# MobilePerceptionLab/EventCalib

Measured on AMD Instinct MI355X. Metric: Mevents/s DBSCAN+detect, higher is better.
Workload: dtype f64; 1 GPU; ONE 50M-event synthetic circle-grid stream (BASELINE configs[2]'s stream), 346x260, 1 Mev/s, tiled 1.5 ms windows (33334 windows), eps 4 minpts 2; stages: window bounds + EventFrame slicing (reference point order) + DBSCAN(+/-) + circle candidates (reference tie picks); HBM-resident when the timed region starts, upload excluded (reported beside: h2d, ingest); events_total=50000000, events_covered_by_the_ranks_windows=50000000, windows_total=33334, events_per_gpu=50000000, windows_per_gpu=33334, unique_points_per_gpu=38558159, max_window_events=1501, max_segment_points=666, windows_reaching_pairing=26228, circle_candidates=839094, event_point=False

## Files before the change

### eventcalib_amd/csrc/ecal_events.hip

```cpp
#include "ecal_ctx.hpp"
#include "slice_order.hpp"
#include "slice_hash.hpp"

#pragma clang fp contract(off)

namespace ecal {


template <bool STRICT>
__device__ __forceinline__ uint64_t bound_search(const uint8_t *__restrict__ rec, uint64_t n, double t, double t_first, double t_last) {
    auto below = [&](uint64_t i) {
        const double v = load_f64_unaligned(rec + i * RECORD_BYTES);
        return STRICT ? (v <= t) : (v < t);
    };
    if (n == 0) return 0;
    const double f = (t - t_first) / (t_last - t_first);
    uint64_t g = f >= 1.0 ? n - 1 : (f > 0.0 ? (uint64_t) (f * (double) (n - 1)) : 0);
    if (g > n - 1) g = n - 1;
    uint64_t lo, hi;
    if (below(g)) {
        lo = g + 1;
        hi = n;
        for (uint64_t w = 32;; w *= 2) {
            const uint64_t p = g + w;
// ... 422 lines not shown
                                                  uint32_t cap_points, double *__restrict__ xy_out,
                                                  uint32_t *__restrict__ seg_off, uint32_t *__restrict__ seg_cnt,
                                                  int32_t *__restrict__ event_point, int *overflow,
                                                  unsigned char *order_scratch) {
    const uint32_t lo = win_lo[s], n = win_hi[s] - lo, base = win_base[s];
    if (n == 0) {
        if (lo_excl == 0 && threadIdx.x == 0) {
            seg_off[2 * s] = base < cap_points ? base : 0;
            seg_off[2 * s + 1] = seg_off[2 * s];
            seg_cnt[2 * s] = 0;
            seg_cnt[2 * s + 1] = 0;
        }
        return;
    }
    if (n <= lo_excl || n > (uint32_t) CAP) return;
    if ((uint64_t) base + n > cap_points) {
        if (threadIdx.x == 0) {
            *overflow = 1;
            seg_off[2 * s] = seg_off[2 * s + 1] = 0;
            seg_cnt[2 * s] = seg_cnt[2 * s + 1] = 0;
        }
        return;
    }
    using L = SliceLayout<CAP>;
    SliceWork<uint16_t> w;
    w.pts = reinterpret_cast<double2 *>(smem + L::pts_off);
    w.bend = reinterpret_cast<uint32_t *>(smem + L::bend_off);
    w.bend_words = CAP + 4;
    w.pts_words = 4 * CAP;
    w.pos = reinterpret_cast<uint32_t *>(smem + L::pos_off);
    w.sorted = reinterpret_cast<uint16_t *>(smem + L::sorted_off);
    w.rep = reinterpret_cast<uint16_t *>(smem + L::rep_off);
    w.pol = reinterpret_cast<uint8_t *>(smem + L::pol_off);
    w.red = reinterpret_cast<uint32_t *>(smem + L::red_off);
    uint32_t nP, nN;
    OrderScratch ord;
    uint32_t *evk = nullptr;
    if (order_scratch) {
        unsigned char *o = order_scratch + (size_t) blockIdx.x * order_scratch_bytes(CAP);
        order_scratch_carve(o, CAP, &ord, &evk);
    }
    slice_window<T, false, uint16_t>(w, rec, lo, n, Log2c<NB>::value, xy_out + 2 * (size_t) base, event_point ? event_point + base : nullptr,
                                     &nP, &nN, order_scratch ? &ord : nullptr, evk);
    if (threadIdx.x == 0) {
        seg_off[2 * s] = base;
        seg_cnt[2 * s] = nP;
        seg_off[2 * s + 1] = base + nP;
        seg_cnt[2 * s + 1] = nN;
    }
}

template <int CAP, int NB, int T>
__global__ __launch_bounds__(T) void slice_lds_kernel(const uint8_t *__restrict__ rec,
                                                      const uint32_t *__restrict__ win_lo,
                                                      const uint32_t *__restrict__ win_hi,
                                                      const uint32_t *__restrict__ win_base, uint32_t lo_excl,
                                                      uint32_t cap_points, double *__restrict__ xy_out,
                                                      uint32_t *__restrict__ seg_off, uint32_t *__restrict__ seg_cnt,
                                                      int32_t *__restrict__ event_point, int *overflow, uint32_t S,
                                                      const uint32_t *__restrict__ todo,
                                                      const uint32_t *__restrict__ todo_count,
                                                      unsigned char *order_scratch ) {
    extern __shared__ __attribute__((aligned(16))) unsigned char smem[];
    const uint32_t count = todo ? *todo_count : S;
    for (uint32_t k = blockIdx.x; k < count; k += gridDim.x) {
        slice_tier_window<CAP, NB, T>(smem, todo ? todo[k] : k, rec, win_lo, win_hi, win_base, lo_excl, cap_points, xy_out,
                                      seg_off, seg_cnt, event_point, overflow, order_scratch);
        __syncthreads();
    }
}

__global__ void bucket_table_kernel(uint2 *__restrict__ tab) {
    const uint32_t pix = blockIdx.x * blockDim.x + threadIdx.x;
    if (pix >= (1u << 21)) return;
    const uint64_t h = ref_hash_combine2(HASH_INT.v[pix >> 10], HASH_INT.v[pix & 0x3FFu]);
    uint2 w;
    w.x = (uint32_t) (h % 257ull) | ((uint32_t) (h % 541ull) << 9) | ((uint32_t) (h % 1109ull) << 19);
    w.y = (uint32_t) (h % 13ull) | ((uint32_t) (h % 29ull) << 4) | ((uint32_t) (h % 59ull) << 9) | ((uint32_t) (h % 127ull) << 15);
    tab[pix] = w;
}


#ifndef ECAL_RO_WAVES
#define ECAL_RO_WAVES 5
#endif
#if ECAL_RO_WAVES
#define ECAL_RO_ATTR __attribute__((amdgpu_waves_per_eu(ECAL_RO_WAVES, ECAL_RO_WAVES)))
#else
#define ECAL_RO_ATTR
#endif
__global__ __launch_bounds__(PXH_T) ECAL_RO_ATTR void slice_hash_ref_kernel(const uint8_t *__restrict__ rec,
                                                           const uint32_t *__restrict__ win_lo,
                                                           const uint32_t *__restrict__ win_hi,
                                                           const uint32_t *__restrict__ win_base, uint32_t cap_points,
                                                           double *__restrict__ xy_out, uint32_t *__restrict__ seg_off,
                                                           uint32_t *__restrict__ seg_cnt,
                                                           int32_t *__restrict__ event_point, int *overflow,
                                                           uint32_t *__restrict__ todo,
                                                           uint32_t *__restrict__ todo_count,
                                                           const uint2 *__restrict__ bucket_tab, uint32_t *__restrict__ xy16,
                                                           uint32_t *__restrict__ seg_fmt) {
    extern __shared__ __attribute__((aligned(16))) unsigned char smem[];
    slice_hash_window<11, true>(smem, blockIdx.x, rec, win_lo, win_hi, win_base, cap_points, xy_out, seg_off, seg_cnt, event_point, overflow,
                                todo, todo_count, bucket_tab, xy16, seg_fmt);
}

__global__ __launch_bounds__(PXH_T) void slice_hash_kernel(const uint8_t *__restrict__ rec,
                                                           const uint32_t *__restrict__ win_lo,
                                                           const uint32_t *__restrict__ win_hi,
                                                           const uint32_t *__restrict__ win_base, uint32_t cap_points,
                                                           double *__restrict__ xy_out, uint32_t *__restrict__ seg_off,
                                                           uint32_t *__restrict__ seg_cnt,
                                                           int32_t *__restrict__ event_point, int *overflow,
                                                           uint32_t *__restrict__ todo,
                                                           uint32_t *__restrict__ todo_count, uint32_t *__restrict__ xy16,
                                                           uint32_t *__restrict__ seg_fmt) {
    extern __shared__ __attribute__((aligned(16))) unsigned char smem[];
    slice_hash_window<11, false>(smem, blockIdx.x, rec, win_lo, win_hi, win_base, cap_points, xy_out, seg_off, seg_cnt, event_point, overflow,
                                 todo, todo_count, nullptr, xy16, seg_fmt);
}

template <bool THIRD >
__global__ __launch_bounds__(PXH_T) __attribute__((amdgpu_waves_per_eu(THIRD ? 2 : 3, THIRD ? 2 : 3))) void slice_hash_ref_both_kernel(const uint8_t *__restrict__ rec, const uint32_t *__restrict__ win_lo,
                                                                    const uint32_t *__restrict__ win_hi, const uint32_t *__restrict__ win_base,
                                                                    uint32_t cap_points, double *__restrict__ xy_out, uint32_t *__restrict__ seg_off,
                                                                    uint32_t *__restrict__ seg_cnt, int32_t *__restrict__ event_point, int *overflow,
                                                                    uint32_t *__restrict__ todo, uint32_t *__restrict__ todo_count,
                                                                    uint32_t *__restrict__ todo2, uint32_t *__restrict__ todo2_count,
                                                                    uint32_t *__restrict__ todo3, uint32_t *__restrict__ todo3_count,
                                                                    const uint2 *__restrict__ bucket_tab, uint32_t *__restrict__ xy16,
                                                                    uint32_t *__restrict__ seg_fmt) {
    extern __shared__ __attribute__((aligned(16))) unsigned char smem[];
    const uint32_t s = blockIdx.x;
    const uint32_t n = win_hi[s] - win_lo[s];
    if constexpr (THIRD) {
        bool done = false;
        if (n <= PixHash<11>::CAP)
            done = slice_hash_window<11, true>(smem, s, rec, win_lo, win_hi, win_base, cap_points, xy_out, seg_off, seg_cnt, event_point, overflow,
                                               nullptr, nullptr, bucket_tab, xy16, seg_fmt);
        if (!done && n <= PixHash<12>::CAP) {
            __syncthreads();
            done = slice_hash_window<12, true>(smem, s, rec, win_lo, win_hi, win_base, cap_points, xy_out, seg_off, seg_cnt, event_point, overflow,
                                               nullptr, nullptr, bucket_tab, xy16, seg_fmt);
        }
        if (!done) {
            __syncthreads();
            slice_hash_window<13, true>(smem, s, rec, win_lo, win_hi, win_base, cap_points, xy_out, seg_off, seg_cnt, event_point, overflow, todo3,
                                        todo3_count, bucket_tab, xy16, seg_fmt);
        }
        return;
    }
    if (n <= PixHash<11>::CAP)
        slice_hash_window<11, true>(smem, s, rec, win_lo, win_hi, win_base, cap_points, xy_out, seg_off, seg_cnt, event_point, overflow, todo,
                                    todo_count, bucket_tab, xy16, seg_fmt);
    else
        slice_hash_window<12, true>(smem, s, rec, win_lo, win_hi, win_base, cap_points, xy_out, seg_off, seg_cnt, event_point, overflow, todo2,
                                    todo2_count, bucket_tab, xy16, seg_fmt);
}

__global__ __launch_bounds__(PXH_T) __attribute__((amdgpu_waves_per_eu(2, 2))) void slice_hash_third_kernel(const uint8_t *__restrict__ rec, const uint32_t *__restrict__ win_lo,
                                                                 const uint32_t *__restrict__ win_hi, const uint32_t *__restrict__ win_base,
                                                                 uint32_t cap_points, double *__restrict__ xy_out, uint32_t *__restrict__ seg_off,
                                                                 uint32_t *__restrict__ seg_cnt, int32_t *__restrict__ event_point, int *overflow,
                                                                 uint32_t *__restrict__ todo, uint32_t *__restrict__ todo_count,
                                                                 const uint32_t *__restrict__ in_list, const uint32_t *__restrict__ in_count,
                                                                 const uint2 *__restrict__ bucket_tab, uint32_t *__restrict__ xy16,
                                                                 uint32_t *__restrict__ seg_fmt) {
// ... 407 lines not shown
```

### eventcalib_amd/csrc/slice_hash.hpp

```cpp
#pragma once
#include "ecal_ctx.hpp"
#include "slice_order.hpp"

#pragma clang fp contract(off)

namespace ecal {

constexpr int RECORD_BYTES = 25;

__device__ __forceinline__ double load_f64_unaligned(const uint8_t *p) {
    double v;
    __builtin_memcpy(&v, p, 8);
    return v;
}

#ifdef ECAL_PHASE_PROF
static __device__ unsigned long long g_ro_cycles[16];
#define RO_MARK(i)                                                                                  \
    do {                                                                                            \
        if (REFORDER && LOGC == 11 && threadIdx.x == 0) {                                           \
            const unsigned long long now__ = __builtin_amdgcn_s_memtime();                          \
            atomicAdd(&g_ro_cycles[i], now__ - ro_t__);                                             \
            ro_t__ = now__;                                                                         \
        }                                                                                           \
    } while (0)
#else
#define RO_MARK(i)
#endif
#ifndef ECAL_RO_STOP
#define ECAL_RO_STOP 0
#endif
#ifndef ECAL_SL_STOP
#define ECAL_SL_STOP 0
#endif

constexpr int PXH_T = 256;
#ifndef ECAL_PXH13_PER
#define ECAL_PXH13_PER 20
#endif
template <int LOGC>
struct PixHash {
    static constexpr uint32_t SLOTS = 1u << LOGC;
    static constexpr int PER = LOGC == 13 ? ECAL_PXH13_PER : (int) (SLOTS / PXH_T);
    static constexpr uint32_t CAP = (uint32_t) PER * PXH_T - 1u;
    static constexpr uint32_t PIXB = 32u - LOGC;
    static constexpr double XMAX = (double) ((1u << (PIXB - 10u)) - 1u), YMAX = 1023.0;
    static constexpr size_t tab_off = 0;
    static constexpr size_t red_off = tab_off + 8 * SLOTS;
    static constexpr size_t bytes = red_off + 16 * 8 + 16;
    static __device__ __forceinline__ uint32_t slot(uint32_t pix) { return (pix * 0x9E3779B1u) >> (32u - LOGC); }
#ifndef ECAL_RO_NI
#define ECAL_RO_NI 9
#endif
#ifndef ECAL_RO_NI2
#define ECAL_RO_NI2 16
#endif
    static constexpr int NI = LOGC == 11 ? ECAL_RO_NI : (LOGC == 12 ? ECAL_RO_NI2 : 19);
    static constexpr int MAX_EPOCHS = LOGC == 11 ? 7 : 8;
    static constexpr uint32_t NOFF = 128u * NI, PSL = 2u * NOFF;
#ifndef ECAL_RO_FA
#define ECAL_RO_FA 2400
#endif
    static constexpr uint32_t FA_CAP = LOGC == 11 ? (uint32_t) ECAL_RO_FA : 4800u;
    static constexpr size_t w_off = 0;
    static constexpr size_t region_off = w_off + 4 * PSL;
    static constexpr size_t cur_off = region_off + 2 * (PSL > SLOTS ? PSL : SLOTS);
    static constexpr size_t fa_off = cur_off + 2 * PSL;
    static constexpr size_t keep_off = fa_off + 4 * FA_CAP;
    static constexpr size_t bcnt_off = keep_off + 4 * 16 * NI;
    static constexpr size_t ored_off = bcnt_off + 4 * (SLOTS / 64 + 4);
    static constexpr size_t obytes = ored_off + 16 * 8 + 16;
};

struct HashIntTable {
    uint64_t v[2048];
    constexpr HashIntTable() : v{} {
        for (int i = 0; i < 2048; i++) v[i] = ref_hash_f64_bits(__builtin_bit_cast(uint64_t, (double) i));
    }
};
static __device__ const HashIntTable HASH_INT = HashIntTable();

struct ModB {
    double b, inv;
};
__host__ __device__ constexpr double ref_step_inv(int e) { return (1.0 / (double) ref_bucket_step(e)) * (1.0 - 0x1p-50); }
struct StepInvTable {
    double inv[12];
    constexpr StepInvTable() : inv{} {
        for (int e = 0; e < 12; e++) inv[e] = ref_step_inv(e);
    }
};
__device__ __forceinline__ ModB mod_for_epoch(int e) {
    constexpr StepInvTable tabl = StepInvTable();
    ModB m;
    m.b = (double) ref_bucket_step(e);
    m.inv = tabl.inv[e];
    return m;
}
__device__ __forceinline__ double mod_step(double v, const ModB m) {
    const double q = __builtin_trunc(v * m.inv);
    double r = __builtin_fma(-q, m.b, v);
    if (r >= m.b) r -= m.b;
    return r;
}
__device__ __forceinline__ uint32_t mod_hash(uint64_t h, const ModB m) {
    const double d1 = (double) (uint32_t) (h >> 40);
    const double d0 = __builtin_fma((double) (uint32_t) ((h >> 32) & 0xFFu), 0x1p32, (double) (uint32_t) h);
    const double r1 = mod_step(d1, m);
    return (uint32_t) mod_step(__builtin_fma(r1, 0x1p40, d0), m);
}

__device__ __forceinline__ void lds_barrier() {
    asm volatile("s_waitcnt lgkmcnt(0)\n\ts_barrier" ::: "memory");
}

__device__ __forceinline__ void wave_sync_lds() {
    __builtin_amdgcn_fence(__ATOMIC_ACQ_REL, "wavefront");
    __builtin_amdgcn_wave_barrier();
}

__device__ __forceinline__ uint32_t wave_incl_scan_dpp(uint32_t x) {
    uint32_t t = x;
    t += (uint32_t) __builtin_amdgcn_update_dpp(0, (int) x, 0x111, 0xF, 0xF, false);
    t += (uint32_t) __builtin_amdgcn_update_dpp(0, (int) x, 0x112, 0xF, 0xF, false);
    t += (uint32_t) __builtin_amdgcn_update_dpp(0, (int) x, 0x113, 0xF, 0xF, false);
    t += (uint32_t) __builtin_amdgcn_update_dpp(0, (int) t, 0x114, 0xF, 0xE, false);
    t += (uint32_t) __builtin_amdgcn_update_dpp(0, (int) t, 0x118, 0xF, 0xC, false);
    t += (uint32_t) __builtin_amdgcn_update_dpp(0, (int) t, 0x142, 0xA, 0xF, false);
    t += (uint32_t) __builtin_amdgcn_update_dpp(0, (int) t, 0x143, 0xC, 0xF, false);
    return t;
}

__device__ __forceinline__ void early_epochs_packed(uint32_t m, uint32_t *fa, uint32_t *W, uint16_t *region, uint16_t *cur_out) {
    const uint32_t lane = threadIdx.x & 63u;
    const uint32_t m_e = m < 127u ? m : 127u;
    uint32_t bw[2], cur[2] = {0u, 0u};
#pragma unroll
    for (int i = 0; i < 2; i++) bw[i] = (lane + 64u * i < m_e) ? fa[lane + 64u * i] : 0u;
    wave_sync_lds();
    uint32_t n_prev = 0;
    for (int e = 0; e < 4 && n_prev < m_e; e++) {
        const uint32_t B = (uint32_t) ref_bucket_step(e);
        const uint32_t n_e = m_e < B ? m_e : B;
        const uint32_t sh = e == 0 ? 0u : (e == 1 ? 4u : (e == 2 ? 9u : 15u)), mask = (16u << e) - 1u;
#pragma unroll
        for (int i = 0; i < 2; i++) {
            if (lane + 64u * i < B) fa[lane + 64u * i] = 0xFFFFFFFFu;
            if (lane + 64u * i < m_e) W[lane + 64u * i] = 0u;
        }
        wave_sync_lds();
        uint32_t b[2], q[2], f[2], sl[2];
#pragma unroll
        for (int i = 0; i < 2; i++) {
            const uint32_t u = lane + 64u * i;
            q[i] = u < n_prev ? cur[i] : u;
            b[i] = (bw[i] >> sh) & mask;
            if (u < n_e) atomicMin(&fa[b[i]], q[i]);
        }
        wave_sync_lds();
#pragma unroll
        for (int i = 0; i < 2; i++) {
            const uint32_t u = lane + 64u * i;
            f[i] = 0;
            sl[i] = 0;
            if (u < n_e) {
                f[i] = fa[b[i]];
                sl[i] = atomicAdd(&W[f[i]], 1u);
            }
        }
        wave_sync_lds();
        {
            const uint32_t c0 = 2u * lane < n_e ? W[2u * lane] : 0u, c1 = 2u * lane + 1u < n_e ? W[2u * lane + 1u] : 0u;
            const uint32_t ex = wave_incl_scan_dpp(c0 + c1) - c0 - c1;
            if (2u * lane < n_e) W[2u * lane] = (ex << 16) | c0;
            if (2u * lane + 1u < n_e) W[2u * lane + 1u] = ((ex + c0) << 16) | c1;
        }
        wave_sync_lds();
#pragma unroll
        for (int i = 0; i < 2; i++) {
            const uint32_t u = lane + 64u * i;
            if (u < n_e) region[(W[f[i]] >> 16) + sl[i]] = (uint16_t) q[i];
        }
        wave_sync_lds();
#pragma unroll
        for (int i = 0; i < 2; i++) {
            const uint32_t u = lane + 64u * i;
            if (u < n_e) {
                const uint32_t w = W[f[i]], b0 = w >> 16, c = w & 0xFFFFu;
                uint32_t within = 0;
                for (uint32_t t = 0; t < c; t++) within += ((uint32_t) region[b0 + t] < q[i]) ? 1u : 0u;
                cur[i] = n_e - 1u - (b0 + within);
            }
        }
        wave_sync_lds();
        n_prev = n_e;
    }
#pragma unroll
    for (int i = 0; i < 2; i++)
        if (lane + 64u * i < m_e) cur_out[lane + 64u * i] = (uint16_t) cur[i];
}

template <int LOGC, bool REFORDER>
__device__ __forceinline__ bool slice_hash_window(unsigned char *smem, const uint32_t s, const uint8_t *__restrict__ rec,
                                                  const uint32_t *__restrict__ win_lo, const uint32_t *__restrict__ win_hi,
                                                  const uint32_t *__restrict__ win_base, uint32_t cap_points,
                                                  double *__restrict__ xy_out, uint32_t *__restrict__ seg_off,
                                                  uint32_t *__restrict__ seg_cnt, int32_t *__restrict__ event_point,
                                                  int *overflow, uint32_t *__restrict__ todo,
                                                  uint32_t *__restrict__ todo_count, const uint2 *__restrict__ bucket_tab = nullptr,
                                                  uint32_t *__restrict__ xy16 = nullptr, uint32_t *__restrict__ seg_fmt = nullptr) {
    using L = PixHash<LOGC>;
    constexpr int T = PXH_T;
#ifdef ECAL_PHASE_PROF
    unsigned long long ro_t__ = __builtin_amdgcn_s_memtime();
#endif
    constexpr uint32_t PXH_CAP = L::CAP, PXH_SLOTS = L::SLOTS, IDXM = L::SLOTS - 1u, PIXB = L::PIXB;
    constexpr uint32_t MB = LOGC <= 12 ? 12u : 13u, M_IDX = (1u << MB) - 1u, M_ER = 1u << MB, M_POL = 2u << MB, M_KEY = 4u << MB;
    static_assert(MB + 3u <= 16u && L::CAP <= M_IDX, "the word's fields");
    constexpr int PXH_PER = L::PER;
    constexpr uint32_t NONE = L::CAP, EMPTY = 0xFFFFFFFFu;
    const uint32_t tid = threadIdx.x;
    const uint32_t lo = win_lo[s], n = win_hi[s] - lo, base = win_base[s];
    if (n == 0) {
        if (tid == 0) {
            seg_off[2 * s] = base < cap_points ? base : 0;
            seg_off[2 * s + 1] = seg_off[2 * s];
            seg_cnt[2 * s] = 0;
            seg_cnt[2 * s + 1] = 0;
            if (seg_fmt) seg_fmt[2 * s] = seg_fmt[2 * s + 1] = 0u;
        }
        return true;
    }
    if (n > PXH_CAP) {
        if (tid == 0) {
            if (todo) todo[atomicAdd(todo_count, 1u)] = s;
            if (seg_fmt) seg_fmt[2 * s] = seg_fmt[2 * s + 1] = 0u;
        }
        return false;
    }
    if ((uint64_t) base + n > cap_points) {
        if (tid == 0) {
            *overflow = 1;
            seg_off[2 * s] = seg_off[2 * s + 1] = 0;
            seg_cnt[2 * s] = seg_cnt[2 * s + 1] = 0;
            if (seg_fmt) seg_fmt[2 * s] = seg_fmt[2 * s + 1] = 0u;
        }
        return true;
    }
    uint32_t *const tab = reinterpret_cast<uint32_t *>(smem + L::tab_off);
    uint16_t *const pos = reinterpret_cast<uint16_t *>(smem + L::tab_off);
    uint32_t *const red = reinterpret_cast<uint32_t *>(smem + L::red_off);
    uint32_t *const badf = red + 32;

    double vx[PXH_PER], vy[PXH_PER];
    uint32_t vp[PXH_PER];
#pragma unroll
    for (int j = 0; j < PXH_PER; j++) {
        const uint32_t k = tid + j * T;
        vx[j] = 0;
        vy[j] = 0;
        vp[j] = 0;
        if (k < n) {
            const uint8_t *r = rec + (uint64_t) (lo + k) * RECORD_BYTES;
            vx[j] = load_f64_unaligned(r + 8);
            vy[j] = load_f64_unaligned(r + 16);
            vp[j] = r[24];
        }
    }
    {
        uint4 *t4 = reinterpret_cast<uint4 *>(tab);
        for (uint32_t q = tid; q < 2 * PXH_SLOTS / 4; q += T) t4[q] = make_uint4(EMPTY, EMPTY, EMPTY, EMPTY);
    }
    bool bad = false;
    uint32_t pix[PXH_PER];
#pragma unroll
    for (int j = 0; j < PXH_PER; j++) {
        const uint32_t k = tid + j * T;
        const double x = vx[j], y = vy[j];
        const bool okc = x == floor(x) && y == floor(y) && x <= L::XMAX && y <= L::YMAX && __double_as_longlong(x) >= 0 &&
                         __double_as_longlong(y) >= 0;
        bad = bad || (k < n && !okc);
        pix[j] = (((uint32_t) (int) x << 10) | ((uint32_t) (int) y & 0x3FFu)) & ((1u << PIXB) - 1u);
    }
    const bool wave_bad = __any(bad);
    if ((tid & 63) == 0) badf[tid >> 6] = wave_bad ? 1u : 0u;
    __syncthreads();
    if (badf[0] | badf[1] | badf[2] | badf[3]) {
        if (tid == 0) {
            if (todo) todo[atomicAdd(todo_count, 1u)] = s;
            if (seg_fmt) seg_fmt[2 * s] = seg_fmt[2 * s + 1] = 0u;
        }
        return false;
    }
    if (ECAL_SL_STOP == 1) return true;
    constexpr bool EARLY_GATHER = REFORDER;
    uint2 bw[EARLY_GATHER ? PXH_PER : 1];
    if constexpr (EARLY_GATHER) {
#pragma unroll
        for (int j = 0; j < PXH_PER; j++) bw[j] = (tid + j * T < n) ? bucket_tab[pix[j]] : make_uint2(0u, 0u);
    }
    uint32_t hs[PXH_PER];
    {
        uint32_t w0[PXH_PER];
#pragma unroll
        for (int j = 0; j < PXH_PER; j++) {
            hs[j] = L::slot(pix[j]);
            w0[j] = tab[(vp[j] ? PXH_SLOTS : 0u) + hs[j]];
        }
#pragma unroll
        for (int j = 0; j < PXH_PER; j++) {
            const uint32_t k = tid + j * T;
            if (k < n) {
                uint32_t *const t = tab + (vp[j] ? PXH_SLOTS : 0u);
                const uint32_t mine = (pix[j] << LOGC) | k;
                uint32_t h = hs[j], w = w0[j];
                for (;;) {
                    if (w == EMPTY) w = atomicCAS(&t[h], EMPTY, mine);
                    if (w == EMPTY) break;
                    if ((w >> LOGC) == pix[j]) {
                        atomicMin(&t[h], mine);
                        break;
                    }
                    h = (h + 1u) & (PXH_SLOTS - 1u);
                    w = t[h];
                }
                hs[j] = h;
            }
        }
    }
    if constexpr (EARLY_GATHER) lds_barrier(); else __syncthreads();
    if (ECAL_SL_STOP == 2) return true;
    uint32_t repk[PXH_PER];
    uint32_t firstk[PXH_PER];
    {
        uint32_t fw[PXH_PER], ow[PXH_PER];
#pragma unroll
        for (int j = 0; j < PXH_PER; j++) {
            fw[j] = tab[(vp[j] ? PXH_SLOTS : 0u) + hs[j]];
            ow[j] = tab[(vp[j] ? 0u : PXH_SLOTS) + L::slot(pix[j])];
        }
#pragma unroll
        for (int j = 0; j < PXH_PER; j++) {
            const uint32_t k = tid + j * T;
            if (k < n) {
                const uint32_t first = fw[j] & IDXM;
                const uint32_t *const o = tab + (vp[j] ? 0u : PXH_SLOTS);
                uint32_t h = L::slot(pix[j]), w = ow[j];
                bool both = false;
                for (;;) {
                    if (w == EMPTY) break;
                    if ((w >> LOGC) == pix[j]) {
                        both = true;
                        break;
                    }
                    h = (h + 1u) & (PXH_SLOTS - 1u);
                    w = o[h];
                }
                repk[j] = both ? NONE : first;
                firstk[j] = first | (both ? 0x8000u : 0u);
            } else {
                repk[j] = NONE;
                firstk[j] = 0xFFFFu;
            }
        }
    }
    if constexpr (EARLY_GATHER) lds_barrier(); else __syncthreads();
    RO_MARK(1);
    if (ECAL_SL_STOP == 3) return true;
    if constexpr (REFORDER) {
        constexpr uint32_t N_EARLY = 127u;
        uint32_t *const W = reinterpret_cast<uint32_t *>(smem + L::w_off);
        uint16_t *const region = reinterpret_cast<uint16_t *>(smem + L::region_off);
        uint16_t *const cur = reinterpret_cast<uint16_t *>(smem + L::cur_off);
        uint32_t *const fa = reinterpret_cast<uint32_t *>(smem + L::fa_off);
        uint32_t *const keepW = reinterpret_cast<uint32_t *>(smem + L::keep_off);
        uint32_t *const ored = reinterpret_cast<uint32_t *>(smem + L::ored_off);
        uint16_t *const posE = region;
        const uint32_t lane = tid & 63u, wave = tid >> 6;
        constexpr uint32_t NBATCH = (uint32_t) PXH_PER * (T / 64);
        uint32_t *const bcnt = reinterpret_cast<uint32_t *>(smem + L::bcnt_off);
        uint32_t meta[PXH_PER];
#pragma unroll
        for (int j = 0; j < PXH_PER; j++) {
            const uint32_t k = tid + j * T;
            const bool isu = k < n && (firstk[j] & 0x7FFFu) == k;
            const unsigned long long mP = __ballot(isu && vp[j] != 0), mN = __ballot(isu && vp[j] == 0);
            const unsigned long long lower = (1ull << lane) - 1ull;
            const uint32_t below = (uint32_t) __popcll((vp[j] ? mP : mN) & lower);
            if (lane == 0) bcnt[j * (T / 64) + wave] = (uint32_t) __popcll(mP) | ((uint32_t) __popcll(mN) << 16);
            meta[j] = k < n ? ((firstk[j] & M_IDX) | ((firstk[j] & 0x8000u) ? M_ER : 0u) | (vp[j] ? M_POL : 0u) |
                               (isu ? M_KEY : 0u) | (below << 16))
                            : M_ER;
        }
        if constexpr (EARLY_GATHER) lds_barrier(); else __syncthreads();
    RO_MARK(2);
        if (tid < 64u) {
            if constexpr (NBATCH <= 64u) {
                const uint32_t v = tid < NBATCH ? bcnt[tid] : 0u;
                uint32_t inc = v;
#pragma unroll
                for (int d = 1; d < 64; d <<= 1) {
                    const uint32_t o = __shfl_up(inc, d, 64);
                    if (lane >= (uint32_t) d) inc += o;
                }
                if (tid < NBATCH) bcnt[tid] = inc - v;
                if (tid == 63u) bcnt[NBATCH] = inc;
            } else {
                static_assert(NBATCH <= 128u, "two batches per lane");
                const uint32_t v0 = 2u * tid < NBATCH ? bcnt[2u * tid] : 0u, v1 = 2u * tid + 1u < NBATCH ? bcnt[2u * tid + 1u] : 0u;
                uint32_t inc = v0 + v1;
#pragma unroll
                for (int d = 1; d < 64; d <<= 1) {
                    const uint32_t o = __shfl_up(inc, d, 64);
                    if (lane >= (uint32_t) d) inc += o;
                }
                if (2u * tid < NBATCH) bcnt[2u * tid] = inc - v0 - v1;
                if (2u * tid + 1u < NBATCH) bcnt[2u * tid + 1u] = inc - v1;
                if (tid == 63u) bcnt[NBATCH] = inc;
            }
        }
        if constexpr (EARLY_GATHER) lds_barrier(); else __syncthreads();
    RO_MARK(3);
        const uint32_t totals = bcnt[NBATCH], mP = totals & 0xFFFFu, mN = totals >> 16;
        const int EP = mP ? ref_epochs(mP) : 0, EN = mN ? ref_epochs(mN) : 0;
        {
            const uint32_t need = (EP ? (uint32_t) ref_bucket_step(EP - 1) : 0u) + (EN ? (uint32_t) ref_bucket_step(EN - 1) : 0u);
            if (need > L::FA_CAP || EP > L::MAX_EPOCHS || EN > L::MAX_EPOCHS || mP > 128u * (uint32_t) L::NI ||
                mN > 128u * (uint32_t) L::NI) {
                if (tid == 0) {
            if (todo) todo[atomicAdd(todo_count, 1u)] = s;
            if (seg_fmt) seg_fmt[2 * s] = seg_fmt[2 * s + 1] = 0u;
        }
                return false;
            }
        }
        {
            constexpr int NI = L::NI;
            const uint32_t faN = EP ? (uint32_t) ref_bucket_step(EP - 1) : 0u;
            {
#pragma unroll
                for (int j = 0; j < PXH_PER; j++) {
                    const uint32_t ex = bcnt[j * (T / 64) + wave];
                    meta[j] += ((meta[j] & M_POL) ? (ex & 0xFFFFu) : (ex >> 16)) << 16;
                    if (meta[j] & M_KEY) {
                        const uint32_t rank = meta[j] >> 16;
                        const bool pos_ = (meta[j] & M_POL) != 0;
                        W[(pos_ ? 0u : L::NOFF) + rank] = bw[j].x | ((meta[j] & M_ER) ? 0x80000000u : 0u);
                        if (rank < N_EARLY) fa[(pos_ ? 0u : faN) + rank] = bw[j].y;
                        if (L::MAX_EPOCHS > 7 && (pos_ ? EP : EN) > 7)
                            region[(pos_ ? 0u : L::NOFF) + rank] =
                                (uint16_t) mod_hash(ref_hash_combine2(HASH_INT.v[pix[j] >> 10], HASH_INT.v[pix[j] & 0x3FFu]), mod_for_epoch(7));
                    }
                }
            }
            if (ECAL_RO_STOP == 2) return true;
            const uint32_t pol = __builtin_amdgcn_readfirstlane(wave >> 1), sub = __builtin_amdgcn_readfirstlane(wave & 1u);
            const uint32_t l128 = lane + 64u * sub;
            const uint32_t m = pol == 0u ? mP : mN;
            const int E = pol == 0u ? EP : EN;
            const uint32_t uoff = pol == 0u ? 0u : L::NOFF;
            uint32_t *const Wp = W + uoff, *const fap = fa + (pol == 0u ? 0u : faN);
            uint16_t *const regp = region + uoff, *const curp = cur + uoff;
            constexpr uint32_t KW = 4u * NI;
            uint32_t *const kW = keepW + pol * KW, *const kPre = keepW + 2u * KW + pol * KW;
            if (tid == 0) ored[10] = 0u;
            __syncthreads();
    RO_MARK(4);
            uint32_t bk[NI], cu[NI];
#pragma unroll
            for (int i = 0; i < NI; i++) {
                const uint32_t u = l128 + 128u * i;
                bk[i] = u < m ? Wp[u] : 0u;
                cu[i] = (L::MAX_EPOCHS > 7 && E > 7 && u < m) ? ((uint32_t) regp[u] << 16) : 0u;
            }
            if (l128 < KW) kW[l128] = 0u;
            __syncthreads();
    RO_MARK(5);
            if (sub == 0u && m) early_epochs_packed(m, fap, Wp, regp, curp);
            __syncthreads();
    RO_MARK(6);
            if (ECAL_RO_STOP == 3) return true;
            if (l128 < (m < 127u ? m : 127u)) cu[0] = (cu[0] & 0xFFFF0000u) | (uint32_t) curp[l128];
            const int EMAX = EP > EN ? EP : EN;
            if (E > 4) {
                for (uint32_t b = l128; b < 257u; b += 128u) fap[b] = 0xFFFFFFFFu;
            }
            __syncthreads();
    RO_MARK(7);
            for (int e = 4; e < EMAX; e++) {
                const bool on = e < E;
                const uint32_t B = (uint32_t) ref_bucket_step(e), Bprev = (uint32_t) ref_bucket_step(e - 1);
                const uint32_t n_e = on ? (m < B ? m : B) : 0u;
                const uint32_t sh = e == 4 ? 0u : (e == 5 ? 9u : (e == 6 ? 19u : 16u)),
                               bmask = e == 4 ? 0x1FFu : (e == 5 ? 0x3FFu : (e == 6 ? 0x7FFu : 0xFFFu));
                const bool e7 = e == 7;
                const uint32_t per = (n_e + 127u) >> 7;
                uint32_t fq[NI];
                for (uint32_t t = 0; t < per; t++) Wp[l128 + 128u * t] = 0u;
#pragma unroll
                for (int i = 0; i < NI; i++) {
                    const uint32_t u = l128 + 128u * i;
                    if (128u * i >= n_e) break;
                    if (u < n_e) atomicMin(&fap[((e7 ? cu[i] : bk[i]) >> sh) & bmask], u < Bprev ? (cu[i] & 0xFFFFu) : u);
                }
                __syncthreads();
#pragma unroll
                for (int i = 0; i < NI; i++) {
                    const uint32_t u = l128 + 128u * i;
                    fq[i] = 0u;
                    if (128u * i >= n_e) break;
                    if (u < n_e) {
                        const uint32_t f = fap[((e7 ? cu[i] : bk[i]) >> sh) & bmask];
                        fq[i] = f | (atomicAdd(&Wp[f], 1u) << 12);
                    }
                }
                __syncthreads();
                {
                    uint32_t c[NI], sum = 0, big = 0;
#pragma unroll
                    for (int t = 0; t < NI; t++) {
                        c[t] = 0u;
                        if ((uint32_t) t < per) c[t] = Wp[l128 * per + t];
                        sum += c[t];
                        big |= c[t];
                    }
                    if (__any(big > 1023u)) ored[10] = 1u;
                    const uint32_t inc = wave_incl_scan_dpp(sum);
                    if (lane == 63u) ored[wave] = inc;
                    uint32_t ex = inc - sum;
#pragma unroll
                    for (int t = 0; t < NI; t++) {
                        if ((uint32_t) t < per) Wp[l128 * per + t] = (ex << 10) | (c[t] & 0x3FFu);
                        ex += c[t];
                    }
                    if (e + 1 < E) {
                        const uint32_t Bn = (uint32_t) ref_bucket_step(e + 1);
                        for (uint32_t b = l128; b < Bn; b += 128u) fap[b] = 0xFFFFFFFFu;
                    }
                }
                __syncthreads();
                const uint32_t carry_from = 64u * per, carry = __builtin_amdgcn_readfirstlane(ored[pol * 2u]);
#pragma unroll
                for (int i = 0; i < NI; i++) {
                    const uint32_t u = l128 + 128u * i;
                    if (128u * i >= n_e) break;
                    if (u < n_e) {
                        const uint32_t f = fq[i] & 0xFFFu, w = Wp[f];
                        if ((w & 0x3FFu) > 2u)
                            regp[(w >> 10) + (f >= carry_from ? carry : 0u) + (fq[i] >> 12)] = (uint16_t) (u < Bprev ? (cu[i] & 0xFFFFu) : u);
                    }
                }
                __syncthreads();
#pragma unroll
                for (int i = 0; i < NI; i++) {
                    const uint32_t u = l128 + 128u * i;
                    if (128u * i >= n_e) break;
                    if (u < n_e) {
                        const uint32_t f = fq[i] & 0xFFFu, w = Wp[f], b0 = (w >> 10) + (f >= carry_from ? carry : 0u), cnt = w & 0x3FFu;
                        const uint32_t q = u < Bprev ? (cu[i] & 0xFFFFu) : u;
                        uint32_t within = (q != f) ? 1u : 0u;
                        if (cnt > 2u) {
                            const uint32_t r0 = regp[b0], r1 = regp[b0 + 1u], r2 = regp[b0 + 2u], r3 = regp[b0 + 3u];
                            within = (r0 < q ? 1u : 0u) + (r1 < q ? 1u : 0u) + (r2 < q ? 1u : 0u) + ((cnt > 3u && r3 < q) ? 1u : 0u);
                            for (uint32_t t = 4; t < cnt; t++) within += ((uint32_t) regp[b0 + t] < q) ? 1u : 0u;
                        }
                        cu[i] = (cu[i] & 0xFFFF0000u) | (n_e - 1u - (b0 + within));
                    }
                }
                __syncthreads();
                RO_MARK(8 + (e - 4));
            }
            if (ECAL_RO_STOP == 4) return true;
            if (ored[10]) {
                if (tid == 0) {
            if (todo) todo[atomicAdd(todo_count, 1u)] = s;
            if (seg_fmt) seg_fmt[2 * s] = seg_fmt[2 * s + 1] = 0u;
        }
                return false;
            }
#pragma unroll
            for (int i = 0; i < NI; i++) {
                const uint32_t u = l128 + 128u * i;
                if (u < m && !(bk[i] >> 31)) atomicOr(&kW[(cu[i] & 0xFFFFu) >> 5], 1u << (cu[i] & 31u));
            }
            __syncthreads();
    RO_MARK(11);
            if (sub == 0u) {
                static_assert(KW <= 128u, "two bitmap words per lane");
                const uint32_t c0 = 2u * lane < KW ? (uint32_t) __popc(kW[2u * lane]) : 0u;
                const uint32_t c1 = 2u * lane + 1u < KW ? (uint32_t) __popc(kW[2u * lane + 1u]) : 0u;
                const uint32_t inc = wave_incl_scan_dpp(c0 + c1);
                if (2u * lane < KW) kPre[2u * lane] = inc - c0 - c1;
                if (2u * lane + 1u < KW) kPre[2u * lane + 1u] = inc - c1;
                if (lane == 63u) ored[8u + pol] = inc;
            }
            __syncthreads();
    RO_MARK(12);
#pragma unroll
            for (int i = 0; i < NI; i++) {
                const uint32_t u = l128 + 128u * i;
                if (u < m && !(bk[i] >> 31))
                    curp[u] = (uint16_t) (kPre[(cu[i] & 0xFFFFu) >> 5] + (uint32_t) __popc(kW[(cu[i] & 0xFFFFu) >> 5] & ((1u << (cu[i] & 31u)) - 1u)));
            }
            __syncthreads();
    RO_MARK(13);
            const uint32_t nP = mP ? __builtin_amdgcn_readfirstlane(ored[8]) : 0u, nN = mN ? __builtin_amdgcn_readfirstlane(ored[9]) : 0u;
            const bool want_ep = event_point != nullptr;
            if (want_ep) {
#pragma unroll
                for (int j = 0; j < PXH_PER; j++) {
                    if ((meta[j] & (M_KEY | M_ER)) == M_KEY)
                        posE[meta[j] & M_IDX] = cur[((meta[j] & M_POL) ? 0u : L::NOFF) + (meta[j] >> 16)];
                }
                __syncthreads();
            }
    RO_MARK(14);
            double2 *out2 = reinterpret_cast<double2 *>(xy_out) + base;
            int32_t *ep = want_ep ? event_point + base : nullptr;
#pragma unroll
            for (int j = 0; j < PXH_PER; j++) {
                const uint32_t k = tid + j * T;
                if (k < n) {
                    if (meta[j] & M_ER) {
                        if (want_ep) ep[k] = -1;
                    } else if (want_ep || (meta[j] & M_KEY)) {
                        const uint32_t at = want_ep ? posE[meta[j] & M_IDX]
                                                    : (uint32_t) cur[((meta[j] & M_POL) ? 0u : L::NOFF) + (meta[j] >> 16)];
                        if (want_ep) ep[k] = (int32_t) at;
                        if (meta[j] & M_KEY) {
                            const uint32_t slot = (meta[j] & M_POL) ? at : nP + at;
                            if (xy16) {
                                xy16[base + slot] = (pix[j] >> 10) | ((pix[j] & 0x3FFu) << 16);
                            } else {
                                double2 v;
                                v.x = (double) (pix[j] >> 10);
                                v.y = (double) (pix[j] & 0x3FFu);
                                out2[slot] = v;
                            }
                        }
                    }
                }
            }
            if (tid == 0) {
                seg_off[2 * s] = base;
                seg_cnt[2 * s] = nP;
                seg_off[2 * s + 1] = base + nP;
                seg_cnt[2 * s + 1] = nN;
                if (seg_fmt) seg_fmt[2 * s] = seg_fmt[2 * s + 1] = xy16 ? 1u : 0u;
            }
            RO_MARK(15);
            RO_MARK(0);
            return true;
        }
    }
    constexpr uint32_t NBATCH = (uint32_t) PXH_PER * (T / 64);
    static_assert(REFORDER || NBATCH <= 64u, "the canonical-order form scans one batch per lane (first and second pass only)");
    uint32_t *const bcnt = tab + PXH_SLOTS;
    const uint32_t lane = tid & 63u, wave = tid >> 6;
    uint32_t below[PXH_PER];
#pragma unroll
    for (int j = 0; j < PXH_PER; j++) {
        const uint32_t k = tid + j * T;
        const bool isrep = k < n && repk[j] == k;
        const unsigned long long mP = __ballot(isrep && vp[j] != 0), mN = __ballot(isrep && vp[j] == 0);
        const unsigned long long lower = (1ull << lane) - 1ull;
        below[j] = (uint32_t) __popcll((vp[j] ? mP : mN) & lower);
        if (lane == 0) bcnt[j * (T / 64) + wave] = (uint32_t) __popcll(mP) | ((uint32_t) __popcll(mN) << 16);
    }
    __syncthreads();
    if (tid < 64u) {
        const uint32_t v = tid < NBATCH ? bcnt[tid] : 0u;
        uint32_t inc = v;
#pragma unroll
        for (int d = 1; d < 64; d <<= 1) {
            const uint32_t o = __shfl_up(inc, d, 64);
            if (lane >= (uint32_t) d) inc += o;
        }
        if (tid < NBATCH) bcnt[tid] = inc - v;
        if (tid == 63u) bcnt[NBATCH] = inc;
    }
    __syncthreads();
    const uint32_t totals = bcnt[NBATCH], nP = totals & 0xFFFFu, nN = totals >> 16;
#pragma unroll
    for (int j = 0; j < PXH_PER; j++) {
        const uint32_t k = tid + j * T;
        if (k < n && repk[j] == k) {
            const uint32_t ex = bcnt[j * (T / 64) + wave];
            pos[k] = (uint16_t) ((vp[j] ? (ex & 0xFFFFu) : (ex >> 16)) + below[j]);
        }
    }
    __syncthreads();
    if (ECAL_SL_STOP == 4) return true;
    double2 *out2 = reinterpret_cast<double2 *>(xy_out) + base;
    int32_t *ep = event_point ? event_point + base : nullptr;
#pragma unroll
    for (int j = 0; j < PXH_PER; j++) {
        const uint32_t k = tid + j * T;
        if (k < n) {
            const uint32_t r = repk[j];
            if (r == NONE) {
                if (ep) ep[k] = -1;
            } else {
                const uint32_t at = pos[r];
                if (ep) ep[k] = (int32_t) at;
                if (r == k) {
                    const uint32_t slot = vp[j] ? at : nP + at;
                    if (xy16) {
                        xy16[base + slot] = (pix[j] >> 10) | ((pix[j] & 0x3FFu) << 16);
                    } else {
                        double2 v;
                        v.x = (double) (pix[j] >> 10);
                        v.y = (double) (pix[j] & 0x3FFu);
                        out2[slot] = v;
                    }
                }
            }
        }
    }
    if (tid == 0) {
        seg_off[2 * s] = base;
        seg_cnt[2 * s] = nP;
        seg_off[2 * s + 1] = base + nP;
        seg_cnt[2 * s + 1] = nN;
        if (seg_fmt) seg_fmt[2 * s] = seg_fmt[2 * s + 1] = xy16 ? 1u : 0u;
    }
    return true;
}
}
```

Measured before the change: 20010 Mevents/s.

## Raise slice pass occupancy: alias LDS buffers, pack polarity, add short-window form

Pushes the first slicing pass from five to six waves per EU and shrinks its LDS footprint so six workgroups fit per CU. The cur array now aliases the W buffer, and the early-epoch positions are placed inside W. Polarity is packed into bit 31 of the pixel word, and two meta slots are stashed to LDS across the long epoch section, both to cut register pressure. A short-form specialization with fewer per-thread slots handles windows under 6*T events. The aliasing is only safe if cur and W lifetimes never overlap, and the stash adds LDS traffic.

```diff
diff --git a/eventcalib_amd/csrc/ecal_events.hip b/eventcalib_amd/csrc/ecal_events.hip
--- a/eventcalib_amd/csrc/ecal_events.hip
+++ b/eventcalib_amd/csrc/ecal_events.hip
@@ -528,7 +528,7 @@
 
 
 #ifndef ECAL_RO_WAVES
-#define ECAL_RO_WAVES 5
+#define ECAL_RO_WAVES 6
 #endif
 #if ECAL_RO_WAVES
 #define ECAL_RO_ATTR __attribute__((amdgpu_waves_per_eu(ECAL_RO_WAVES, ECAL_RO_WAVES)))
diff --git a/eventcalib_amd/csrc/slice_hash.hpp b/eventcalib_amd/csrc/slice_hash.hpp
--- a/eventcalib_amd/csrc/slice_hash.hpp
+++ b/eventcalib_amd/csrc/slice_hash.hpp
@@ -64,13 +64,19 @@
     static constexpr uint32_t FA_CAP = LOGC == 11 ? (uint32_t) ECAL_RO_FA : 4800u;
     static constexpr size_t w_off = 0;
     static constexpr size_t region_off = w_off + 4 * PSL;
-    static constexpr size_t cur_off = region_off + 2 * (PSL > SLOTS ? PSL : SLOTS);
-    static constexpr size_t fa_off = cur_off + 2 * PSL;
+    static constexpr size_t cur_off = w_off;
+    static constexpr size_t ecur_off = 4 * 128;
+    static_assert(ecur_off + 2 * 128 <= 4 * NOFF, "the early epochs' positions lie inside the set's part of W");
+    static_assert(cur_off + 2 * PSL <= region_off, "cur lies inside W (every LOGC): nothing sits between region and fa any more");
+    static constexpr size_t fa_off = region_off + 2 * (PSL > SLOTS ? PSL : SLOTS);
     static constexpr size_t keep_off = fa_off + 4 * FA_CAP;
     static constexpr size_t bcnt_off = keep_off + 4 * 16 * NI;
     static constexpr size_t ored_off = bcnt_off + 4 * (SLOTS / 64 + 4);
-    static constexpr size_t obytes = ored_off + 16 * 8 + 16;
+    static constexpr int NSTASH = LOGC == 11 ? 2 : 0, STASH0 = 4;
+    static constexpr size_t stash_off = ored_off + 16 * 8 + 16;
+    static constexpr size_t obytes = stash_off + 4 * NSTASH * PXH_T;
 };
+static_assert(6 * PixHash<11>::obytes <= 163840 && PixHash<11>::obytes <= 27136, "first pass: six workgroups per CU");
 
 struct HashIntTable {
     uint64_t v[2048];
@@ -200,15 +206,15 @@
         if (lane + 64u * i < m_e) cur_out[lane + 64u * i] = (uint16_t) cur[i];
 }
 
-template <int LOGC, bool REFORDER>
-__device__ __forceinline__ bool slice_hash_window(unsigned char *smem, const uint32_t s, const uint8_t *__restrict__ rec,
-                                                  const uint32_t *__restrict__ win_lo, const uint32_t *__restrict__ win_hi,
-                                                  const uint32_t *__restrict__ win_base, uint32_t cap_points,
-                                                  double *__restrict__ xy_out, uint32_t *__restrict__ seg_off,
-                                                  uint32_t *__restrict__ seg_cnt, int32_t *__restrict__ event_point,
-                                                  int *overflow, uint32_t *__restrict__ todo,
-                                                  uint32_t *__restrict__ todo_count, const uint2 *__restrict__ bucket_tab = nullptr,
-                                                  uint32_t *__restrict__ xy16 = nullptr, uint32_t *__restrict__ seg_fmt = nullptr) {
+template <int LOGC, bool REFORDER, int PER>
+__device__ __forceinline__ bool slice_hash_window_slots(unsigned char *smem, const uint32_t s, const uint8_t *__restrict__ rec,
+                                                        const uint32_t *__restrict__ win_lo, const uint32_t *__restrict__ win_hi,
+                                                        const uint32_t *__restrict__ win_base, uint32_t cap_points,
+                                                        double *__restrict__ xy_out, uint32_t *__restrict__ seg_off,
+                                                        uint32_t *__restrict__ seg_cnt, int32_t *__restrict__ event_point,
+                                                        int *overflow, uint32_t *__restrict__ todo,
+                                                        uint32_t *__restrict__ todo_count, const uint2 *__restrict__ bucket_tab,
+                                                        uint32_t *__restrict__ xy16, uint32_t *__restrict__ seg_fmt) {
     using L = PixHash<LOGC>;
     constexpr int T = PXH_T;
 #ifdef ECAL_PHASE_PROF
@@ -217,7 +223,8 @@
     constexpr uint32_t PXH_CAP = L::CAP, PXH_SLOTS = L::SLOTS, IDXM = L::SLOTS - 1u, PIXB = L::PIXB;
     constexpr uint32_t MB = LOGC <= 12 ? 12u : 13u, M_IDX = (1u << MB) - 1u, M_ER = 1u << MB, M_POL = 2u << MB, M_KEY = 4u << MB;
     static_assert(MB + 3u <= 16u && L::CAP <= M_IDX, "the word's fields");
-    constexpr int PXH_PER = L::PER;
+    static_assert(PER >= 1 && PER <= L::PER, "a short form of the pass: fewer slots, the same tables and limits");
+    constexpr int PXH_PER = PER;
     constexpr uint32_t NONE = L::CAP, EMPTY = 0xFFFFFFFFu;
     const uint32_t tid = threadIdx.x;
     const uint32_t lo = win_lo[s], n = win_hi[s] - lo, base = win_base[s];
@@ -271,6 +278,10 @@
         uint4 *t4 = reinterpret_cast<uint4 *>(tab);
         for (uint32_t q = tid; q < 2 * PXH_SLOTS / 4; q += T) t4[q] = make_uint4(EMPTY, EMPTY, EMPTY, EMPTY);
     }
+    constexpr uint32_t POLB = 0x80000000u, PIXM = (1u << PIXB) - 1u;
+    static_assert(PIXB < 31u, "bit 31 of the pixel word is free");
+#define PIX_OF(w) ((w) & PIXM)
+#define POL_OF(w) (((w) & POLB) != 0u)
     bool bad = false;
     uint32_t pix[PXH_PER];
 #pragma unroll
@@ -280,7 +291,7 @@
         const bool okc = x == floor(x) && y == floor(y) && x <= L::XMAX && y <= L::YMAX && __double_as_longlong(x) >= 0 &&
                          __double_as_longlong(y) >= 0;
         bad = bad || (k < n && !okc);
-        pix[j] = (((uint32_t) (int) x << 10) | ((uint32_t) (int) y & 0x3FFu)) & ((1u << PIXB) - 1u);
+        pix[j] = ((((uint32_t) (int) x << 10) | ((uint32_t) (int) y & 0x3FFu)) & PIXM) | (vp[j] ? POLB : 0u);
     }
     const bool wave_bad = __any(bad);
     if ((tid & 63) == 0) badf[tid >> 6] = wave_bad ? 1u : 0u;
@@ -297,27 +308,27 @@
     uint2 bw[EARLY_GATHER ? PXH_PER : 1];
     if constexpr (EARLY_GATHER) {
 #pragma unroll
-        for (int j = 0; j < PXH_PER; j++) bw[j] = (tid + j * T < n) ? bucket_tab[pix[j]] : make_uint2(0u, 0u);
+        for (int j = 0; j < PXH_PER; j++) bw[j] = (tid + j * T < n) ? bucket_tab[PIX_OF(pix[j])] : make_uint2(0u, 0u);
     }
     uint32_t hs[PXH_PER];
     {
         uint32_t w0[PXH_PER];
 #pragma unroll
         for (int j = 0; j < PXH_PER; j++) {
-            hs[j] = L::slot(pix[j]);
-            w0[j] = tab[(vp[j] ? PXH_SLOTS : 0u) + hs[j]];
+            hs[j] = L::slot(PIX_OF(pix[j]));
+            w0[j] = tab[(POL_OF(pix[j]) ? PXH_SLOTS : 0u) + hs[j]];
         }
 #pragma unroll
         for (int j = 0; j < PXH_PER; j++) {
             const uint32_t k = tid + j * T;
             if (k < n) {
-                uint32_t *const t = tab + (vp[j] ? PXH_SLOTS : 0u);
+                uint32_t *const t = tab + (POL_OF(pix[j]) ? PXH_SLOTS : 0u);
                 const uint32_t mine = (pix[j] << LOGC) | k;
                 uint32_t h = hs[j], w = w0[j];
                 for (;;) {
                     if (w == EMPTY) w = atomicCAS(&t[h], EMPTY, mine);
                     if (w == EMPTY) break;
-                    if ((w >> LOGC) == pix[j]) {
+                    if ((w >> LOGC) == PIX_OF(pix[j])) {
                         atomicMin(&t[h], mine);
                         break;
                     }
@@ -336,20 +347,20 @@
         uint32_t fw[PXH_PER], ow[PXH_PER];
 #pragma unroll
         for (int j = 0; j < PXH_PER; j++) {
-            fw[j] = tab[(vp[j] ? PXH_SLOTS : 0u) + hs[j]];
-            ow[j] = tab[(vp[j] ? 0u : PXH_SLOTS) + L::slot(pix[j])];
+            fw[j] = tab[(POL_OF(pix[j]) ? PXH_SLOTS : 0u) + hs[j]];
+            ow[j] = tab[(POL_OF(pix[j]) ? 0u : PXH_SLOTS) + L::slot(PIX_OF(pix[j]))];
         }
 #pragma unroll
         for (int j = 0; j < PXH_PER; j++) {
             const uint32_t k = tid + j * T;
             if (k < n) {
                 const uint32_t first = fw[j] & IDXM;
-                const uint32_t *const o = tab + (vp[j] ? 0u : PXH_SLOTS);
-                uint32_t h = L::slot(pix[j]), w = ow[j];
+                const uint32_t *const o = tab + (POL_OF(pix[j]) ? 0u : PXH_SLOTS);
+                uint32_t h = L::slot(PIX_OF(pix[j])), w = ow[j];
                 bool both = false;
                 for (;;) {
                     if (w == EMPTY) break;
-                    if ((w >> LOGC) == pix[j]) {
+                    if ((w >> LOGC) == PIX_OF(pix[j])) {
                         both = true;
                         break;
                     }
@@ -384,11 +395,12 @@
         for (int j = 0; j < PXH_PER; j++) {
             const uint32_t k = tid + j * T;
             const bool isu = k < n && (firstk[j] & 0x7FFFu) == k;
-            const unsigned long long mP = __ballot(isu && vp[j] != 0), mN = __ballot(isu && vp[j] == 0);
+            const bool pol_ = POL_OF(pix[j]);
+            const unsigned long long mP = __ballot(isu && pol_), mN = __ballot(isu && !pol_);
             const unsigned long long lower = (1ull << lane) - 1ull;
-            const uint32_t below = (uint32_t) __popcll((vp[j] ? mP : mN) & lower);
+            const uint32_t below = (uint32_t) __popcll((pol_ ? mP : mN) & lower);
             if (lane == 0) bcnt[j * (T / 64) + wave] = (uint32_t) __popcll(mP) | ((uint32_t) __popcll(mN) << 16);
-            meta[j] = k < n ? ((firstk[j] & M_IDX) | ((firstk[j] & 0x8000u) ? M_ER : 0u) | (vp[j] ? M_POL : 0u) |
+            meta[j] = k < n ? ((firstk[j] & M_IDX) | ((firstk[j] & 0x8000u) ? M_ER : 0u) | (pol_ ? M_POL : 0u) |
                                (isu ? M_KEY : 0u) | (below << 16))
                             : M_ER;
         }
@@ -449,10 +461,13 @@
                         if (rank < N_EARLY) fa[(pos_ ? 0u : faN) + rank] = bw[j].y;
                         if (L::MAX_EPOCHS > 7 && (pos_ ? EP : EN) > 7)
                             region[(pos_ ? 0u : L::NOFF) + rank] =
-                                (uint16_t) mod_hash(ref_hash_combine2(HASH_INT.v[pix[j] >> 10], HASH_INT.v[pix[j] & 0x3FFu]), mod_for_epoch(7));
-                    }
-                }
-            }
+                                (uint16_t) mod_hash(ref_hash_combine2(HASH_INT.v[PIX_OF(pix[j]) >> 10], HASH_INT.v[pix[j] & 0x3FFu]), mod_for_epoch(7));
+                    }
+                }
+            }
+            uint32_t *const stash = reinterpret_cast<uint32_t *>(smem + L::stash_off);
+#pragma unroll
+            for (int j = L::STASH0; j < L::STASH0 + L::NSTASH && j < PXH_PER; j++) stash[(j - L::STASH0) * T + tid] = meta[j];
             if (ECAL_RO_STOP == 2) return true;
             const uint32_t pol = __builtin_amdgcn_readfirstlane(wave >> 1), sub = __builtin_amdgcn_readfirstlane(wave & 1u);
             const uint32_t l128 = lane + 64u * sub;
@@ -461,6 +476,7 @@
             const uint32_t uoff = pol == 0u ? 0u : L::NOFF;
             uint32_t *const Wp = W + uoff, *const fap = fa + (pol == 0u ? 0u : faN);
             uint16_t *const regp = region + uoff, *const curp = cur + uoff;
+            uint16_t *const ecurp = reinterpret_cast<uint16_t *>(reinterpret_cast<unsigned char *>(Wp) + L::ecur_off);
             constexpr uint32_t KW = 4u * NI;
             uint32_t *const kW = keepW + pol * KW, *const kPre = keepW + 2u * KW + pol * KW;
             if (tid == 0) ored[10] = 0u;
@@ -476,11 +492,11 @@
             if (l128 < KW) kW[l128] = 0u;
             __syncthreads();
     RO_MARK(5);
-            if (sub == 0u && m) early_epochs_packed(m, fap, Wp, regp, curp);
+            if (sub == 0u && m) early_epochs_packed(m, fap, Wp, regp, ecurp);
             __syncthreads();
     RO_MARK(6);
             if (ECAL_RO_STOP == 3) return true;
-            if (l128 < (m < 127u ? m : 127u)) cu[0] = (cu[0] & 0xFFFF0000u) | (uint32_t) curp[l128];
+            if (l128 < (m < 127u ? m : 127u)) cu[0] = (cu[0] & 0xFFFF0000u) | (uint32_t) ecurp[l128];
             const int EMAX = EP > EN ? EP : EN;
             if (E > 4) {
                 for (uint32_t b = l128; b < 257u; b += 128u) fap[b] = 0xFFFFFFFFu;
@@ -579,6 +595,8 @@
                 return false;
             }
 #pragma unroll
+            for (int j = L::STASH0; j < L::STASH0 + L::NSTASH && j < PXH_PER; j++) meta[j] = stash[(j - L::STASH0) * T + tid];
+#pragma unroll
             for (int i = 0; i < NI; i++) {
                 const uint32_t u = l128 + 128u * i;
                 if (u < m && !(bk[i] >> 31)) atomicOr(&kW[(cu[i] & 0xFFFFu) >> 5], 1u << (cu[i] & 31u));
@@ -630,10 +648,10 @@
                         if (meta[j] & M_KEY) {
                             const uint32_t slot = (meta[j] & M_POL) ? at : nP + at;
                             if (xy16) {
-                                xy16[base + slot] = (pix[j] >> 10) | ((pix[j] & 0x3FFu) << 16);
+                                xy16[base + slot] = (PIX_OF(pix[j]) >> 10) | ((pix[j] & 0x3FFu) << 16);
                             } else {
                                 double2 v;
-                                v.x = (double) (pix[j] >> 10);
+                                v.x = (double) (PIX_OF(pix[j]) >> 10);
                                 v.y = (double) (pix[j] & 0x3FFu);
                                 out2[slot] = v;
                             }
@@ -662,9 +680,10 @@
     for (int j = 0; j < PXH_PER; j++) {
         const uint32_t k = tid + j * T;
         const bool isrep = k < n && repk[j] == k;
-        const unsigned long long mP = __ballot(isrep && vp[j] != 0), mN = __ballot(isrep && vp[j] == 0);
+        const bool pol_ = POL_OF(pix[j]);
+        const unsigned long long mP = __ballot(isrep && pol_), mN = __ballot(isrep && !pol_);
         const unsigned long long lower = (1ull << lane) - 1ull;
-        below[j] = (uint32_t) __popcll((vp[j] ? mP : mN) & lower);
+        below[j] = (uint32_t) __popcll((pol_ ? mP : mN) & lower);
         if (lane == 0) bcnt[j * (T / 64) + wave] = (uint32_t) __popcll(mP) | ((uint32_t) __popcll(mN) << 16);
     }
     __syncthreads();
@@ -686,7 +705,7 @@
         const uint32_t k = tid + j * T;
         if (k < n && repk[j] == k) {
             const uint32_t ex = bcnt[j * (T / 64) + wave];
-            pos[k] = (uint16_t) ((vp[j] ? (ex & 0xFFFFu) : (ex >> 16)) + below[j]);
+            pos[k] = (uint16_t) ((POL_OF(pix[j]) ? (ex & 0xFFFFu) : (ex >> 16)) + below[j]);
         }
     }
     __syncthreads();
@@ -704,12 +723,12 @@
                 const uint32_t at = pos[r];
                 if (ep) ep[k] = (int32_t) at;
                 if (r == k) {
-                    const uint32_t slot = vp[j] ? at : nP + at;
+                    const uint32_t slot = POL_OF(pix[j]) ? at : nP + at;
                     if (xy16) {
-                        xy16[base + slot] = (pix[j] >> 10) | ((pix[j] & 0x3FFu) << 16);
+                        xy16[base + slot] = (PIX_OF(pix[j]) >> 10) | ((pix[j] & 0x3FFu) << 16);
                     } else {
                         double2 v;
-                        v.x = (double) (pix[j] >> 10);
+                        v.x = (double) (PIX_OF(pix[j]) >> 10);
                         v.y = (double) (pix[j] & 0x3FFu);
                         out2[slot] = v;
                     }
@@ -725,5 +744,29 @@
         if (seg_fmt) seg_fmt[2 * s] = seg_fmt[2 * s + 1] = xy16 ? 1u : 0u;
     }
     return true;
-}
-}
+#undef PIX_OF
+#undef POL_OF
+}
+
+constexpr int PXH_SHORT_PER = 6;
+template <int LOGC, bool REFORDER>
+__device__ __forceinline__ bool slice_hash_window(unsigned char *smem, const uint32_t s, const uint8_t *__restrict__ rec,
+                                                  const uint32_t *__restrict__ win_lo, const uint32_t *__restrict__ win_hi,
+                                                  const uint32_t *__restrict__ win_base, uint32_t cap_points,
+                                                  double *__restrict__ xy_out, uint32_t *__restrict__ seg_off,
+                                                  uint32_t *__restrict__ seg_cnt, int32_t *__restrict__ event_point,
+                                                  int *overflow, uint32_t *__restrict__ todo,
+                                                  uint32_t *__restrict__ todo_count, const uint2 *__restrict__ bucket_tab = nullptr,
+                                                  uint32_t *__restrict__ xy16 = nullptr, uint32_t *__restrict__ seg_fmt = nullptr) {
+    if constexpr (LOGC == 11) {
+        static_assert(PXH_SHORT_PER < PixHash<11>::PER, "the short form");
+        if (win_hi[s] - win_lo[s] < (uint32_t) PXH_SHORT_PER * PXH_T)
+            return slice_hash_window_slots<11, REFORDER, PXH_SHORT_PER>(smem, s, rec, win_lo, win_hi, win_base, cap_points, xy_out, seg_off,
+                                                                        seg_cnt, event_point, overflow, todo, todo_count, bucket_tab, xy16,
+                                                                        seg_fmt);
+    }
+    return slice_hash_window_slots<LOGC, REFORDER, PixHash<LOGC>::PER>(smem, s, rec, win_lo, win_hi, win_base, cap_points, xy_out, seg_off,
+                                                                       seg_cnt, event_point, overflow, todo, todo_count, bucket_tab, xy16,
+                                                                       seg_fmt);
+}
+}
```

Result: faster. 20770 Mevents/s, median of 6 (+3.8%).
